# ucsd-hdsi-dvs/V2CE-Toolbox

Measured on AMD Instinct MI355X. Metric: frame-pairs/sec end-to-end (UNet+LDATI), 346x260, higher is better.
Workload: dtype f32-as-f16x2 (operands split hi/lo in fp16, 3 MFMAs per product, f32 accumulate)

## Files before the change

### v2ce-toolbox_amd/csrc/conv3d_wt.hip

```cpp
#include "conv3d_dev.h"
#include "conv3d_host.h"

#include <algorithm>
#include <cstdlib>
#include <map>
#include <mutex>
#include <tuple>
#include <vector>

namespace v2ce {
namespace {

constexpr int kWtSlot = 256;
constexpr int kWtChs = 4 * kWtSlot;
constexpr int kWtTaps = 36;

template <int CO_FR, int PO_FR, int RES, bool TAIL = false>
__global__ __launch_bounds__(512, 1) void conv3d_wt_kernel(ConvParams P) {
#if defined(__HIP_DEVICE_COMPILE__)
    [[maybe_unused]] unsigned long long t_all = TICK(), t_bar = 0, t_epi = 0, t_xbar = 0, t_cvt = 0, t_e0 = 0, t_e1 = 0, t_e2 = 0;
    static_assert(PO_FR == 4, "the output transform hands position fragment f to consumer wave f");
    constexpr bool PEPI = !TAIL;
    constexpr int CK = 16, NA = 3, CO_TILE = CO_FR * 32, chs = kWtChs;
    f16x8 *pieces = reinterpret_cast<f16x8 *>(conv_smem);
    float *aff = reinterpret_cast<float *>(conv_smem + (size_t)2 * 4 * chs * 16);

    const int tid = threadIdx.x, lane = tid & 63, l32 = lane & 31, half = lane >> 5;
    const int wave = __builtin_amdgcn_readfirstlane(tid >> 6);
    const int CG = P.Cin / CK;
    const long long wplane = (long long)kWtTaps * CG * P.Cout * 16;

    struct TileId { int b, co_t, t0, h0, w0, s0; };
    auto decode = [&](int vb, TileId &T) -> bool {
        const int xcd = vb & 7, q = vb >> 3;
        T.co_t = P.xcd_remap == 2 ? q / P.per_xcd : q % P.n_co_tiles;
        const int sp = P.xcd_remap == 2 ? q - T.co_t * P.per_xcd : q / P.n_co_tiles;
        int bid = xcd * P.per_xcd + sp;
        if (sp >= P.per_xcd || bid >= P.n_spatial) return false;
        const int iw = bid % P.nW;            bid /= P.nW;
        const int ih = bid % P.nH;            bid /= P.nH;
        const int it = bid % P.nT;            bid /= P.nT;
        T.b = bid;
        T.t0 = it * P.TT; T.h0 = ih * P.TH; T.w0 = iw * P.TW; T.s0 = 0;
        if (P.flat) { T.s0 = iw * P.flat; T.h0 = T.s0 / P.Wout; T.w0 = 0; }
        return true;
    };
    auto pos_of = [&](int m, const TileId &T, int &pp, int &th, int &tw) -> bool {
        if (P.flat) {
            pp = m / P.flat;
            const int s = T.s0 + (m - pp * P.flat);
            const int h = s / P.Wout;
            th = h - T.h0;
            tw = s - h * P.Wout;
            return m < P.n_pos && s < P.Hout * P.Wout;
        }
        pp = m / (P.TH * P.TW);
        const int rem = m - pp * (P.TH * P.TW);
        th = rem / P.TW;
        tw = rem - th * P.TW;
        return m < P.n_pos;
    };
    auto next_tile = [&](int &vb, TileId &T) -> bool {
        for (; vb < P.total_blocks; vb += (int)gridDim.x)
            if (decode(vb, T)) return true;
        return false;
    };

    const float *tail = reinterpret_cast<const float *>(P.wq + 2 * wplane);
    const float w_scale = tail[1];
    auto amax_of = [&](int b) -> float { return P.x0_absmax ? P.x0_absmax[b * P.amax_bs] : 4094.0f; };
    auto scale_of = [&](int b) -> float { return P.x0_absmax ? pow2_prescale(2.0f * amax_of(b)) : 0.5f * kActScale; };
    const int NTB = TAIL ? P.tCG / 4 : 0;
    const int CGT = CG + NTB;
    auto tamax_of = [&](int b) -> float {
        if (!P.tx0_absmax) return 4094.0f;
        float am = P.tx0_absmax[b * P.amax_bs];
        if (P.tx1_absmax) am = fmaxf(am, P.tx1_absmax[b * P.amax_bs]);
        return am;
    };
    auto tscale_of = [&](int b) -> float { return P.tx0_absmax ? pow2_prescale(tamax_of(b)) : kActScale; };
    const float wt_scale = TAIL ? reinterpret_cast<const float *>(P.sc_w + 2 * (long long)P.tCG * P.Cout * 16)[1] : 1.0f;
    auto acc_scale_of = [&](int b) -> float { return TAIL ? fminf(scale_of(b) * w_scale, tscale_of(b) * wt_scale) : scale_of(b) * w_scale; };
    auto xs_of = [&](int b) -> float { return TAIL ? acc_scale_of(b) / w_scale : scale_of(b); };
    auto ts_of = [&](int b) -> float { return acc_scale_of(b) / wt_scale; };
    const int nI = CG < NTB ? CG : NTB;
    auto is_tail = [&](int k) -> bool { return TAIL && (k < 2 * nI ? (k & 1) != 0 : NTB > CG); };
    auto idx_of = [&](int k) -> int { return !TAIL ? k : (k < 2 * nI ? k >> 1 : k - nI); };
    if (P.guard && blockIdx.x == 0 && wave == 0) {
        float sm = 0.0f;
        for (int co = lane; co < P.Cout; co += 64) sm = fmaxf(sm, fabsf(P.scale[co]));
#pragma unroll
        for (int o = 32; o; o >>= 1) sm = fmaxf(sm, __shfl_xor(sm, o));
        const int nb = P.amax_bs ? P.B : 1;
        for (int b = lane; b < nb; b += 64) {
            const float am = 2.0f * amax_of(b), xs = xs_of(b);
            float E = sm * (float)(P.Cin * 27) * 0x1p-25f * (tail[0] / xs + am / tail[1]);
            if (TAIL) {
                const float *tl = reinterpret_cast<const float *>(P.sc_w + 2 * (long long)P.tCG * P.Cout * 16);
                const float tam = tamax_of(b), txs = ts_of(b);
                E += sm * (float)(P.tCG * 16) * 0x1p-25f * (tl[0] / txs + tam / tl[1]);
                if (!(xs > 0x1p-100f && txs > 0x1p-100f)) E = __builtin_inff();
            }
            P.guard[b * P.amax_bs] = E;
        }
    }

    int vb = blockIdx.x;
    TileId T;
    if (!next_tile(vb, T)) return;
    int gc = 0;
    struct Pos { int pp, th, tw; bool ok; };
    auto pos_cached = [&](int m) -> Pos {
        Pos q{0, 0, 0, false};
        if (!P.flat) q.ok = pos_of(m, T, q.pp, q.th, q.tw);
        return q;
    };
    auto pos_get = [&](const Pos &c, int m, const TileId &L) -> Pos {
        if (!P.flat) return c;
        Pos q;
        q.ok = pos_of(m, L, q.pp, q.th, q.tw);
        return q;
    };

    if (wave >= 4) {
        const int ptid = tid - 256;
        const bool wave_on = (wave - 4) * 64 < P.plane;
        const int e_pp = ptid / (P.HH * P.HWd), e_hh = (ptid - e_pp * (P.HH * P.HWd)) / P.HWd, e_hw = ptid - e_pp * (P.HH * P.HWd) - e_hh * P.HWd;
        const Pos tpos = pos_cached(ptid & 127);
        float x_scale = xs_of(T.b);
        float t_scale = TAIL ? ts_of(T.b) : 1.0f;
        TileId Tprev = T;
        unsigned toff[2][2];
        [[maybe_unused]] int tm_pp = 0, tm_hi = 0, tm_wi = 0, tm_hs = 0, tm_ws = 0;
        [[maybe_unused]] bool tm_ok = false;
        __amdgpu_buffer_rsrc_t rs_t0 = __builtin_amdgcn_make_buffer_rsrc(const_cast<float *>(P.x0), 0, 0, 0x00020000), rs_t1 = rs_t0;
        unsigned goff[4];
        float R0[4][CK], R1[4][CK];
        __amdgpu_buffer_rsrc_t rs_in = __builtin_amdgcn_make_buffer_rsrc(const_cast<float *>(P.x0), 0, 0, 0x00020000);
        const long long seq = (long long)P.T * P.Cin * (P.Hin * P.Winp);
        const int cg_bytes = P.Hin * P.Winp * 64;
        auto load_chunk = [&](const TileId &L, int kseq, float (&R)[4][CK]) {
            const int cidx = idx_of(kseq);
            if (is_tail(kseq)) {
                typedef float f32x4g __attribute__((ext_vector_type(4)));
                if (cidx == 0) {
#pragma unroll
                    for (int sidx = 0; sidx < 2; ++sidx) toff[sidx][0] = toff[sidx][1] = kOOB;
                    if (tm_ok) {
                        {
                            const int hi = tm_hi, wi = tm_wi, hs = tm_hs, ws = tm_ws, pp = tm_pp;
#pragma unroll
                            for (int i = 0; i < 2; ++i) {
                                const int t = L.t0 + 2 * pp + i;
                                if (t < P.T) {
                                    toff[0][i] = 4u * (unsigned)((t * P.tC0) * (P.tH0 * P.tW0p)) + 64u * (unsigned)(hs * P.tW0p + ws);
                                    toff[1][i] = 4u * (unsigned)((t * P.tC1) * (P.tHin * P.tWinp)) + 64u * (unsigned)(hi * P.tWinp + wi);
                                }
                            }
                        }
                    }
                    const long long seq0 = (long long)P.T * P.tC0 * (P.tH0 * P.tW0p), seq1 = (long long)P.T * P.tC1 * (P.tHin * P.tWinp);
                    rs_t0 = __builtin_amdgcn_make_buffer_rsrc(const_cast<float *>(P.tx0 + L.b * seq0), 0, (int)(seq0 * 4), 0x00020000);
                    rs_t1 = __builtin_amdgcn_make_buffer_rsrc(const_cast<float *>(P.tx1 ? P.tx1 + L.b * seq1 : P.tx0), 0, P.tx1 ? (int)(seq1 * 4) : 0, 0x00020000);
                }
                const int gs = (wave - 4) >> 1;
                const int CG0 = P.tC0 / 16;
#pragma unroll
                for (int hb = 0; hb < 2; ++hb) {
                    const int g = hb * (P.tCG / 2) + 2 * cidx + gs;
                    const bool s1 = g >= CG0;
                    const int gbytes = s1 ? (g - CG0) * (P.tHin * P.tWinp * 64) : g * (P.tH0 * P.tW0p * 64);
#pragma unroll
                    for (int i = 0; i < 2; ++i)
#pragma unroll
                        for (int k4 = 0; k4 < CK / 4; ++k4) {
                            const f32x4g v = s1 ? __builtin_bit_cast(f32x4g, __builtin_amdgcn_raw_buffer_load_b128(rs_t1, toff[1][i], gbytes + 16 * k4, 0))
                                                : __builtin_bit_cast(f32x4g, __builtin_amdgcn_raw_buffer_load_b128(rs_t0, toff[0][i], gbytes + 16 * k4, 0));
                            R[2 * hb + i][4 * k4] = v[0]; R[2 * hb + i][4 * k4 + 1] = v[1]; R[2 * hb + i][4 * k4 + 2] = v[2]; R[2 * hb + i][4 * k4 + 3] = v[3];
                        }
                }
                return;
            }
            if (cidx == 0) {
                if constexpr (TAIL) {
                    const Pos q = pos_get(tpos, ptid & 127, L);
                    tm_ok = q.ok && L.h0 + q.th < P.Hout && L.w0 + q.tw < P.Wout;
                    tm_pp = q.pp;
                    tm_hi = tm_ok ? (L.h0 + q.th) * P.tS : 0;
                    tm_wi = tm_ok ? (L.w0 + q.tw) * P.tS : 0;
                    tm_hs = P.thmap ? P.thmap[tm_hi] : tm_hi;
                    tm_ws = P.twmap ? P.twmap[tm_wi] : tm_wi;
                }
#pragma unroll
                for (int i = 0; i < 4; ++i) goff[i] = kOOB;
                if (ptid < P.plane) {
                    const int pp = e_pp, hh = e_hh, hw = e_hw;
                    const int h = L.h0 - 1 + hh, w = L.w0 - 1 + hw;
                    if (h >= 0 && h < P.Hin && w >= 0 && w < P.Win) {
#pragma unroll
                        for (int i = 0; i < 4; ++i) {
                            const int t = L.t0 + 2 * pp - 1 + i;
                            if (t >= 0 && t < P.T) goff[i] = 4u * (unsigned)((t * P.Cin) * (P.Hin * P.Winp)) + 64u * (unsigned)(h * P.Winp + w);
                        }
                    }
                }
                rs_in = __builtin_amdgcn_make_buffer_rsrc(const_cast<float *>(P.x0 + L.b * seq), 0, (int)(seq * 4), 0x00020000);
            }
            if (wave_on) {
                typedef float f32x4g __attribute__((ext_vector_type(4)));
#pragma unroll
                for (int i = 0; i < 4; ++i)
#pragma unroll
                    for (int k4 = 0; k4 < CK / 4; ++k4) {
#if defined(V2CE_ABLATE_TAPS) && (V2CE_ABLATE_TAPS & 4)
                        if (k4) { R[i][4 * k4] = R[i][0]; R[i][4 * k4 + 1] = R[i][1]; R[i][4 * k4 + 2] = R[i][2]; R[i][4 * k4 + 3] = R[i][3]; continue; }
#endif
                        const f32x4g v = __builtin_bit_cast(f32x4g, __builtin_amdgcn_raw_buffer_load_b128(rs_in, goff[i], cidx * cg_bytes + 16 * k4, 0));
                        R[i][4 * k4] = v[0]; R[i][4 * k4 + 1] = v[1]; R[i][4 * k4 + 2] = v[2]; R[i][4 * k4 + 3] = v[3];
                    }
            }
        };
        int vbL = vb, cgL = 0;
        TileId TL = T;
        bool moreL = true;
        auto load_next = [&](float (&R)[4][CK]) {
            if (!moreL) return;
            load_chunk(TL, cgL, R);
            if (++cgL == CGT) {
                cgL = 0;
                vbL += (int)gridDim.x;
                moreL = next_tile(vbL, TL);
            }
        };
        int cgC = 0;
        auto convert_with = [&](float c_scale0, float c_scale12, auto tf) __attribute__((always_inline)) {
            f16x8 *qb = pieces + (gc & 1) * 4 * chs;
#pragma unroll
            for (int j = 0; j < 4; ++j) {
                const float c_scale = (j == 1 || j == 2) ? c_scale12 : c_scale0;
#pragma unroll
                for (int hg = 0; hg < 2; ++hg) {
                    typedef unsigned u32x4c __attribute__((ext_vector_type(4)));
                    u32x4c ph, pl;
#pragma unroll
                    for (int c2 = 0; c2 < 4; ++c2) {
                        const float xa = tf(j, 8 * hg + 2 * c2), xb = tf(j, 8 * hg + 2 * c2 + 1);
                        unsigned h, l;
                        asm("v_fma_mixlo_f16 %0, %2, %4, 0\n\t"
                            "v_fma_mixhi_f16 %0, %3, %4, 0\n\t"
                            "v_fma_mixlo_f16 %1, %2, %4, -%0 op_sel_hi:[0,0,1]\n\t"
                            "v_fma_mixhi_f16 %1, %3, %4, -%0 op_sel:[0,0,1] op_sel_hi:[0,0,1]"
                            : "=&v"(h), "=&v"(l) : "v"(xa), "v"(xb), "v"(c_scale));
                        ph[c2] = h;
                        pl[c2] = l;
                    }
                    qb[hg * chs + j * kWtSlot + ptid] = __builtin_bit_cast(f16x8, ph);
                    qb[(2 + hg) * chs + j * kWtSlot + ptid] = __builtin_bit_cast(f16x8, pl);
                }
            }
        };
        auto convert = [&](const float (&R)[4][CK]) {
            const bool tail = is_tail(cgC);
            if (!wave_on && !tail) return;
            [[maybe_unused]] const unsigned long long tcv = TICK();
            if (tail) {
                convert_with(t_scale, 0.5f * t_scale, [&](int j, int c) -> float {
                    return j == 0 ? R[0][c] : j == 1 ? R[2][c] + R[3][c] : j == 2 ? R[2][c] - R[3][c] : -R[1][c];
                });
            } else {
                convert_with(x_scale, x_scale, [&](int j, int c) -> float {
                    return j == 0 ? R[0][c] - R[2][c] : j == 1 ? R[1][c] + R[2][c] : j == 2 ? R[2][c] - R[1][c] : R[1][c] - R[3][c];
                });
            }
            ACC_T(t_cvt, tcv);
        };
        bool moreC = true;
        auto advance = [&]() {
            ++gc;
            if (++cgC == CGT) {
                cgC = 0;
                Tprev = T;
                vb += (int)gridDim.x;
                moreC = next_tile(vb, T);
                if (moreC) {
                    x_scale = xs_of(T.b);
                    if (TAIL) t_scale = ts_of(T.b);
                }
            }
        };
        const int fr = wave - 4;
        int spk;
        {
            const Pos q = pos_cached(fr * 32 + l32);
            spk = q.ok ? (q.pp << 20) | (q.th << 10) | q.tw : -1;
        }
        int seen_b = -1;
        unsigned seen_max = 0u;
        int ntile_p = 0;
        auto tile_rendezvous = [&]() {
            [[maybe_unused]] const unsigned long long tb = TICK();
            if constexpr (!PEPI) {
#pragma unroll
                for (int k = 0; k < 2 * CO_FR; ++k) lds_barrier();
                ACC_T(t_xbar, tb);
                return;
            }
            typedef float f32x4t __attribute__((ext_vector_type(4)));
            typedef unsigned u32x4t __attribute__((ext_vector_type(4)));
            const TileId &E = Tprev;
            const int co0 = E.co_t * CO_TILE;
            const float out_inv_scale = 1.0f / acc_scale_of(E.b);
            const float *a2 = aff + (ntile_p & 1) * 2 * CO_TILE;
            ++ntile_p;
            int poff[2], roff[2];
            {
                const int m = fr * 32 + l32;
// ... 202 lines not shown
        if constexpr (TAIL) {
#pragma unroll
            for (int f = 0; f < PO_FR; ++f) bpt[f] = half * chs + wave * kWtSlot + f * 32 + l32;
        }
        auto chunk_barrier = [&]() -> const f16x8 * {
            const f16x8 *qb = pieces + (gc & 1) * 4 * chs;
            [[maybe_unused]] const unsigned long long tb = TICK();
            __syncthreads();
            ACC_T(t_bar, tb);
            ++gc;
            return qb;
        };
        auto main_chunk = [&](int cg) __attribute__((always_inline)) {
            const f16x8 *qb = chunk_barrier();
                const int wc = slot_off + cg * cg_stride;
                const int wn = cg + 1 < CG ? wc + cg_stride : slot_off;
#pragma unroll
                for (int f = 0; f < PO_FR; ++f) {
                    bh[f] = qb[bhb[f]];
                    bl[f] = qb[bhb[f] + 2 * chs];
                }
                step_loop<0, 9>([&](auto tc) {
                    constexpr int tap = decltype(tc)::value;
                    constexpr int nt = tap + 1;
                    constexpr int dh = nt / 3, dw = nt % 3;
                    constexpr int pt = tap + NA - 1;
#if !(defined(V2CE_ABLATE_TAPS) && (V2CE_ABLATE_TAPS & 1))
                    if constexpr (pt < 9) {
                        V2CE_LOAD_A(pt % NA, wc + pt * tap_stride)
                    } else {
                        V2CE_LOAD_A(pt % NA, wn + (pt - 9) * tap_stride)
                    }
#endif
                    const int toff = dh * P.HWd + dw;
#pragma unroll
                    for (int f = 0; f < PO_FR; ++f) {
#pragma unroll
                        for (int q = 0; q < CO_FR; ++q) {
                            acc[q][f] = __builtin_amdgcn_mfma_f32_32x32x16_f16(ah[tap % NA][q], bh[f], acc[q][f], 0, 0, 0);
                            acc[q][f] = __builtin_amdgcn_mfma_f32_32x32x16_f16(ah[tap % NA][q], bl[f], acc[q][f], 0, 0, 0);
                            acc[q][f] = __builtin_amdgcn_mfma_f32_32x32x16_f16(al[tap % NA][q], bh[f], acc[q][f], 0, 0, 0);
                        }
#if !(defined(V2CE_ABLATE_TAPS) && (V2CE_ABLATE_TAPS & 2))
                        if constexpr (nt < 9) {
                            bh[f] = qb[bhb[f] + toff];
                            bl[f] = qb[bhb[f] + toff + 2 * chs];
                        }
#endif
                        __builtin_amdgcn_sched_barrier(0);
                    }
                });
        };
        auto tail_prefetch = [&](int kb) __attribute__((always_inline)) {
            const int w0 = (gbase + 2 * kb) * cg_stride;
#pragma unroll
            for (int q = 0; q < (TAIL ? CO_FR : 0); ++q) {
                ath[0][q] = __builtin_bit_cast(f16x8, __builtin_amdgcn_raw_buffer_load_b128(rs_t, wlane[q], w0, 0));
                atl[0][q] = __builtin_bit_cast(f16x8, __builtin_amdgcn_raw_buffer_load_b128(rs_t, wlane[q], w0 + (int)(2 * tplane), 0));
            }
        };
        auto tail_barrier = [&](int kb) __attribute__((always_inline)) {
            if constexpr (TAIL) {
                const f16x8 *qb = chunk_barrier();
                const int w1 = (gbase + 2 * kb + 1) * cg_stride;
#pragma unroll
                for (int q = 0; q < CO_FR; ++q) {
                    ath[1][q] = __builtin_bit_cast(f16x8, __builtin_amdgcn_raw_buffer_load_b128(rs_t, wlane[q], w1, 0));
                    atl[1][q] = __builtin_bit_cast(f16x8, __builtin_amdgcn_raw_buffer_load_b128(rs_t, wlane[q], w1 + (int)(2 * tplane), 0));
                }
#pragma unroll
                for (int gs = 0; gs < 2; ++gs) {
#pragma unroll
                    for (int f = 0; f < PO_FR; ++f) {
                        bh[f] = qb[bpt[f] + gs * 128];
                        bl[f] = qb[bpt[f] + gs * 128 + 2 * chs];
                    }
#pragma unroll
                    for (int f = 0; f < PO_FR; ++f)
#pragma unroll
                        for (int q = 0; q < CO_FR; ++q) {
                            acc[q][f] = __builtin_amdgcn_mfma_f32_32x32x16_f16(ath[gs][q], bh[f], acc[q][f], 0, 0, 0);
                            acc[q][f] = __builtin_amdgcn_mfma_f32_32x32x16_f16(ath[gs][q], bl[f], acc[q][f], 0, 0, 0);
                            acc[q][f] = __builtin_amdgcn_mfma_f32_32x32x16_f16(atl[gs][q], bh[f], acc[q][f], 0, 0, 0);
                        }
                }
            }
        };
        if constexpr (!TAIL) {
            for (int cg = 0; cg < CG; ++cg) main_chunk(cg);
        } else {
            for (int i = 0; i < nI; ++i) {
                main_chunk(i);
                tail_prefetch(i);
                tail_barrier(i);
            }
            for (int i = nI; i < CG; ++i) main_chunk(i);
            for (int i = nI; i < NTB; ++i) {
                tail_prefetch(i);
                tail_barrier(i);
            }
        }

        if constexpr (PEPI) {
        [[maybe_unused]] const unsigned long long te = TICK();
        typedef float f32x4t __attribute__((ext_vector_type(4)));
        f32x4t *xch = reinterpret_cast<f32x4t *>(pieces + ((gc - 1) & 1) * 4 * chs);
#pragma unroll
        for (int q = 0; q < CO_FR; ++q) {
#pragma unroll
            for (int f = 0; f < PO_FR; ++f)
#pragma unroll
                for (int r4 = 0; r4 < 4; ++r4) {
                    f32x4t v;
                    v[0] = acc[q][f][4 * r4]; v[1] = acc[q][f][4 * r4 + 1]; v[2] = acc[q][f][4 * r4 + 2]; v[3] = acc[q][f][4 * r4 + 3];
                    xch[f * chs + wave * kWtSlot + r4 * 64 + lane] = v;
                }
            [[maybe_unused]] const unsigned long long tb = TICK();
            lds_barrier();
            lds_barrier();
            ACC_T(t_xbar, tb);
        }
        ACC_T(t_epi, te);
        } else {
        const float *aff_c = aff + ((ntile - 1) & 1) * 2 * CO_TILE;
// ... 94 lines not shown
                    ACC_T(t_xbar, tb);
                    te2 = TICK();
                }
#pragma unroll
                for (int rr = 0; rr < 2; ++rr) {
                    const int r4 = 2 * hp + rr;
#pragma unroll
                    for (int o = 0; o < 2; ++o) {
                        f32x4t out;
#pragma unroll
                        for (int k = 0; k < 4; ++k) {
                            const float y = o == 0 ? (mm[rr][0][k] + mm[rr][1][k]) + mm[rr][2][k] : (mm[rr][1][k] - mm[rr][2][k]) - mm[rr][3][k];
                            float v = y * (scq[r4][k] * inv_scale) + shq[r4][k];
                            v += rv[o][r4][k];
                            v = apply_act(v, slope);
                            out[k] = v;
                            const unsigned av = __builtin_bit_cast(unsigned, v) & vmask[o];
                            ymax = av > ymax ? av : ymax;
                        }
                        __builtin_amdgcn_raw_buffer_store_b128(__builtin_bit_cast(u32x4t, out), rs_y, vo[o], soff(r4), 0);
                        asm volatile("s_nop 1" : "+v"(out));
                    }
                }
            }
        }
        if (P.y_absmax) {
#pragma unroll
            for (int o = 32; o; o >>= 1) {
                const unsigned other = (unsigned)__shfl_xor((int)ymax, o);
                ymax = other > ymax ? other : ymax;
            }
            if (T.b != seen_b) { seen_b = T.b; seen_max = 0u; }
            if (ymax > seen_max) {
                seen_max = ymax;
                if (lane == 0) atomicMax(reinterpret_cast<unsigned *>(P.y_absmax + T.b * P.amax_bs), ymax);
            }
        }
        ACC_T(t_epi, te);
        ACC_T(t_e2, te2);
        }
        vb += (int)gridDim.x;
        more = next_tile(vb, T);
    }
#ifdef V2CE_STAMP
    if (lane == 0 && wave == 0) {
        unsigned long long *o = P.stamps + ((long long)blockIdx.x * 2 + 0) * 8;
        o[0] = TICK() - t_all; o[1] = t_bar; o[2] = t_xbar; o[3] = t_epi; o[4] = (unsigned long long)gc; o[5] = t_e0; o[6] = t_e1; o[7] = t_e2;
    }
#endif
#undef V2CE_LOAD_A
#endif
}

constexpr int kWtMaxBatch = 16;
struct WtLayer {
    const float *w, *sigma;
    _Float16 *packed;
    int rows, cin;
    int cin_total, ci0;
    long long tail_halves;
};
struct WtBatch {
    WtLayer L[kWtMaxBatch];
    int n;
    int blk[kWtMaxBatch + 1];
};
constexpr size_t kWtPackLds = (size_t)32 * 432 * 4 + (size_t)2 * kWtTaps * 514 * 2;

template <int PASS>
__global__ __launch_bounds__(512) void wt_pack_kernel(WtBatch B) {
    extern __shared__ __attribute__((aligned(16))) unsigned char wt_smem[];
    float *wf = reinterpret_cast<float *>(wt_smem);
    _Float16 *hi = reinterpret_cast<_Float16 *>(wt_smem + 32 * 432 * 4), *lo = hi + kWtTaps * 514;
    int l = 0;
    while (l + 1 < B.n && (int)blockIdx.x >= B.blk[l + 1]) ++l;
    const WtLayer &P = B.L[l];
    const int CG = P.cin / 16;
    const int blk = blockIdx.x - B.blk[l];
    const int cg = blk % CG, co0 = (blk / CG) * 32;
    const long long n = (long long)P.rows * P.cin * kWtTaps;
    float *tail = reinterpret_cast<float *>(P.packed + P.tail_halves);
    const float sigma = P.sigma ? P.sigma[0] : 1.0f;
    for (int e = threadIdx.x; e < 32 * 432; e += 512) {
        const int col = e / 432, rem = e - col * 432;
        wf[e] = P.w[((long long)(co0 + col) * P.cin_total + P.ci0 + cg * 16) * 27 + rem] / sigma;
    }
    __syncthreads();
    const float w_scale = PASS ? pow2_prescale(tail[0]) : 1.0f;
    if (PASS && blk == 0 && threadIdx.x == 0) tail[1] = w_scale;
    float m = 0.0f;
    for (int it = threadIdx.x; it < 32 * 16 * 9; it += 512) {
        const int col = it / 144, rem = it - col * 144, j = rem / 9, t9 = rem - j * 9;
        const float *g = wf + col * 432 + j * 27 + t9;
        const float g0 = g[0], g1 = g[9], g2 = g[18];
        float G[4];
        G[0] = g0;
        G[1] = ((g0 + g1) + g2) * 0.5f;
        G[2] = ((g0 - g1) + g2) * 0.5f;
        G[3] = g2;
        if (!PASS) {
            m = fmaxf(m, fmaxf(fabsf(g0), fmaxf(fabsf(g1), fabsf(g2))));
            continue;
        }
#pragma unroll
        for (int s = 0; s < 4; ++s) {
            const float v = G[s] * w_scale;
// ... 30 lines not shown
    if (B.blk[B.n] == 0) return V2CE_OK;
    if (pass == 0) hipLaunchKernelGGL(wt_pack_kernel<0>, dim3(B.blk[B.n]), dim3(512), kWtPackLds, st, B);
    else hipLaunchKernelGGL(wt_pack_kernel<1>, dim3(B.blk[B.n]), dim3(512), kWtPackLds, st, B);
    V2CE_HIP_CHECK(hipGetLastError());
    return V2CE_OK;
}

struct WtBox { int pp, th, tw, flat; };

WtBox choose_wt_box(int B, int T, int H, int W, int n_co, int n_cu, int pos_tile) {
    if (const char *e = getenv("V2CE_WT_BOX")) {
        WtBox b{0, 0, 0, 0};
        if (sscanf(e, "%d,%d,%d", &b.pp, &b.th, &b.tw) == 3 && b.pp > 0 && b.th > 0 && b.tw > 0 && b.pp * b.th * b.tw <= pos_tile &&
            b.pp * (b.th + 2) * (b.tw + 2) <= kWtSlot)
            return b;
    }
    static std::mutex mu;
    static std::map<std::tuple<int, int, int, int, int, int>, WtBox> cache;
    std::lock_guard<std::mutex> g(mu);
    const auto key = std::make_tuple(B, T, H, W, n_co, pos_tile);
    auto it = cache.find(key);
    if (it != cache.end()) return it->second;
    const int pairs = (T + 1) / 2;
    WtBox best{0, 0, 0, 0};
    double best_cost = 1e30;
    for (int pp = 1; pp <= pairs && pp <= 16; ++pp) {
        const int n_max = pos_tile / pp;
        if (n_max < 1) break;
        const int nR = (H * W + n_max - 1) / n_max, n = (H * W + nR - 1) / nR;
        const int rows = std::min(H, (W - 1 + n - 1) / W + 1);
        if (pp * (rows + 2) * (W + 2) > kWtSlot) continue;
        const long long nsp = (long long)B * ((pairs + pp - 1) / pp) * nR;
        const long long blocks = 8 * ((nsp + 7) / 8) * n_co;
        const double rounds = (double)((blocks + n_cu - 1) / n_cu);
        const double halo = (double)pp * (rows + 2) * (W + 2) / kWtSlot;
        const double cost = rounds * (1.0 + 0.15 * halo) + 1e-3 * (double)blocks / n_cu;
        if (cost < best_cost) { best_cost = cost; best = WtBox{pp, rows, W, n}; }
    }
    for (int pp = 1; pp <= pairs && pp <= 16; ++pp)
        for (int th = 1; th <= H && th <= 64; ++th)
            for (int tw = 1; tw <= W && tw <= 128; ++tw) {
                if (pp * th * tw > pos_tile || pp * (th + 2) * (tw + 2) > kWtSlot) continue;
                const long long nsp = (long long)B * ((pairs + pp - 1) / pp) * ((H + th - 1) / th) * ((W + tw - 1) / tw);
                const long long blocks = 8 * ((nsp + 7) / 8) * n_co;
                const double rounds = (double)((blocks + n_cu - 1) / n_cu);
                const double halo = (double)pp * (th + 2) * (tw + 2) / kWtSlot;
                const double cost = rounds * (1.0 + 0.15 * halo) + 1e-3 * (double)blocks / n_cu;
                if (cost < best_cost - 1e-9) { best_cost = cost; best = WtBox{pp, th, tw, 0}; }
            }
    cache.emplace(key, best);
    return best;
}

template <int CO_FR, int PO_FR, int RES, bool TAIL = false>
int launch_wt(ConvParams P, const v2ce_conv3d_desc &d, hipStream_t stream) {
    constexpr int CO_TILE = CO_FR * 32, POS_TILE = PO_FR * 32;
    if (g_name_out) {
        snprintf(g_name_out, g_name_cap, "conv3d_wt_kernel<%d,%d,%d,%d>", CO_FR, PO_FR, RES, (int)TAIL);
        return V2CE_OK;
    }
    P.n_co_tiles = (d.Cout + CO_TILE - 1) / CO_TILE;
    WtBox bx{d.tile_t / 2, d.tile_h, d.tile_w, 0};
    if (bx.pp <= 0 || bx.th <= 0 || bx.tw <= 0) bx = choose_wt_box(d.B, d.T, d.Hout, d.Wout, P.n_co_tiles, persistent_cu_count(), POS_TILE);
    V2CE_REQUIRE(bx.pp > 0 && bx.th > 0 && bx.tw > 0, V2CE_ERR_UNSUPPORTED, "v2ce_conv3d_fwd_wt: no box fits");
    P.TT = 2 * bx.pp; P.TH = bx.th; P.TW = bx.tw;
    P.flat = bx.flat;
    P.n_pos = bx.flat ? bx.pp * bx.flat : bx.pp * bx.th * bx.tw;
    P.HT = bx.pp; P.HH = bx.th + 2; P.HWd = bx.tw + 2;
    P.plane = P.HT * P.HH * P.HWd;
    P.nT = (d.T + P.TT - 1) / P.TT; P.nH = (d.Hout + bx.th - 1) / bx.th; P.nW = (d.Wout + bx.tw - 1) / bx.tw;
    if (bx.flat) { P.nH = 1; P.nW = (d.Hout * d.Wout + bx.flat - 1) / bx.flat; }
    V2CE_REQUIRE(P.n_pos <= POS_TILE && P.plane <= kWtSlot, V2CE_ERR_UNSUPPORTED, "v2ce_conv3d_fwd_wt: tile does not fit");
    P.n_spatial = d.B * P.nT * P.nH * P.nW;
    P.per_xcd = (P.n_spatial + 7) / 8;
    const double w_bytes = (double)CO_TILE * P.Cin * kWtTaps * 4, x_bytes = (double)P.per_xcd * P.n_pos * 2 * P.Cin * 4;
    P.xcd_remap = P.n_co_tiles > 1 && w_bytes * P.n_co_tiles > x_bytes ? 2 : 1;
    const long long blocks = (long long)8 * P.per_xcd * P.n_co_tiles;
    P.total_blocks = (int)blocks;
    const size_t lds = (size_t)kWtChs * (2 * 4 * 16) + 2 * 2 * CO_TILE * sizeof(float);
    auto kern = conv3d_wt_kernel<CO_FR, PO_FR, RES, TAIL>;
    static const int once = [&] {
        (void)hipFuncSetAttribute(reinterpret_cast<const void *>(kern), hipFuncAttributeMaxDynamicSharedMemorySize, (int)lds);
        return 0;
    }();
    (void)once;
    if (getenv("V2CE_WT_VERBOSE"))
        fprintf(stderr, "[wt<%d,%d,%d%s> %dx%dx%dx%d C %d -> %d] box %d pairs x %d x %d%s (%d of %d positions, %d halo elements), %lld tiles\n", CO_FR, PO_FR, RES, TAIL ? ",tail" : "", d.B, d.T,
                d.Hout, d.Wout, P.Cin, P.Cout, bx.pp, bx.th, bx.tw, bx.flat ? " rows: flat ranges" : "", P.n_pos, POS_TILE, P.plane, blocks);
    const unsigned grid = persistent_grid(blocks);
#ifdef V2CE_STAMP
    V2CE_HIP_CHECK(hipMalloc(&P.stamps, (size_t)grid * 16 * sizeof(unsigned long long)));
    V2CE_HIP_CHECK(hipMemset(P.stamps, 0, (size_t)grid * 16 * sizeof(unsigned long long)));
#endif
    hipLaunchKernelGGL(kern, dim3(grid), dim3(512), lds, stream, P);
    V2CE_HIP_CHECK(hipGetLastError());
#ifdef V2CE_STAMP
    {
        std::vector<unsigned long long> h((size_t)grid * 16);
        V2CE_HIP_CHECK(hipDeviceSynchronize());
        V2CE_HIP_CHECK(hipMemcpy(h.data(), P.stamps, h.size() * 8, hipMemcpyDeviceToHost));
        V2CE_HIP_CHECK(hipFree(P.stamps));
        auto mean = [&](int role, int a) {
            double sm = 0;
            for (unsigned k = 0; k < grid; ++k) sm += (double)h[((size_t)k * 2 + role) * 8 + a];
            return sm / grid;
        };
        const double tot = mean(0, 0), chunks = mean(0, 4), tiles = chunks / (P.Cin / 16);
        fprintf(stderr, "[stamp wt<%d,%d,%d> C %d -> %d %dx%d box %dx%dx%d] per workgroup: %.1f tiles, %.0f chunks, %.0f cycles (s_memtime, 100 MHz) | consumer: chunk barriers %.1f %%, "
                "epilogue %.1f %% (its barriers %.1f %%), main loop %.1f %% = %.1f ticks per chunk | producer: chunk barriers %.1f %%, rendezvous %.1f %%, convert %.1f %%\n",
                CO_FR, PO_FR, RES, P.Cin, P.Cout, d.Hout, d.Wout, bx.pp, bx.th, bx.tw, tiles, chunks, tot, 100 * mean(0, 1) / tot, 100 * mean(0, 3) / tot,
                100 * mean(0, 2) / tot, 100 * (tot - mean(0, 1) - mean(0, 3)) / tot, (tot - mean(0, 1) - mean(0, 3)) / chunks, 100 * mean(1, 1) / mean(1, 0),
                100 * mean(1, 2) / mean(1, 0), 100 * mean(1, 3) / mean(1, 0));
        fprintf(stderr, "    epilogue per tile (cycles): loads + dump (incl. the previous round's compute and stores) %.0f, first barrier .. reads %.0f, last compute + stores + range %.0f, barriers %.0f\n",
                mean(0, 5) / tiles, mean(0, 6) / tiles, mean(0, 7) / tiles, mean(0, 2) / tiles);
    }
#endif
    return V2CE_OK;
}

struct WtTail {
    const v2ce_conv3d_desc *desc;
    const float *tx0, *tx1;
    const int *thmap, *twmap;
    const void *w;
    const float *tx0_absmax, *tx1_absmax;
    int res_h, res_wp;
};

int wt_dispatch(const v2ce_conv3d_desc *desc, const float *x, const void *w_wt, const float *scale, const float *shift,
                const float *residual, float *y, const float *x_absmax, float *y_absmax, v2ce_stream_t stream, const WtTail *tl = nullptr) {
    clear_error();
    V2CE_REQUIRE(desc && (g_name_out || (x && w_wt && scale && shift && y)), V2CE_ERR_BAD_ARG, "v2ce_conv3d_fwd_wt: null pointer");
    const v2ce_conv3d_desc &d = *desc;
    V2CE_REQUIRE(d.B > 0 && d.T > 0 && d.C0 > 0 && d.C1 == 0 && d.Hin > 0 && d.Win > 0 && d.Cout > 0, V2CE_ERR_BAD_ARG,
                 "v2ce_conv3d_fwd_wt: bad shape (one source: C1 must be 0)");
    V2CE_REQUIRE(d.ksize == 3 && d.stride_hw == 1 && d.precision == V2CE_PRECISION_F16X2 && d.layout == V2CE_LAYOUT_C16, V2CE_ERR_UNSUPPORTED,
                 "v2ce_conv3d_fwd_wt: a split-half 3x3x3 stride-1 conv on channels-last-16 activations");
    V2CE_REQUIRE(d.H0 == d.Hin && d.W0 == d.Win && d.Hout == d.Hin && d.Wout == d.Win, V2CE_ERR_BAD_ARG, "v2ce_conv3d_fwd_wt: input and output planes must have one size");
    V2CE_REQUIRE(d.C0 % 16 == 0 && d.Cout % 64 == 0, V2CE_ERR_UNSUPPORTED, "v2ce_conv3d_fwd_wt: Cin must be a multiple of 16, Cout of 64");
    V2CE_REQUIRE(d.act >= 0 && d.act <= 2, V2CE_ERR_BAD_ARG, "v2ce_conv3d_fwd_wt: act %d", d.act);
    V2CE_REQUIRE(g_name_out || (aligned16(x, w_wt, residual, y) && (!tl || aligned16(tl->tx0, tl->tx1, tl->w))), V2CE_ERR_BAD_ARG,
                 "v2ce_conv3d_fwd_wt: weight buffers and channels-last-16 tensors must be 16-byte aligned");
    const int Winp = d.W0_pitch > 0 ? d.W0_pitch : d.W0, Woutp = d.Wout_pitch > 0 ? d.Wout_pitch : d.Wout;
    V2CE_REQUIRE(Winp >= d.Win && Woutp >= d.Wout, V2CE_ERR_BAD_ARG, "v2ce_conv3d_fwd_wt: a row pitch is smaller than its width");
    V2CE_REQUIRE((long long)d.T * d.C0 * d.Hin * Winp < (1ll << 29) && (long long)d.T * d.Cout * d.Hout * Woutp < (1ll << 29), V2CE_ERR_UNSUPPORTED,
                 "v2ce_conv3d_fwd_wt: a single sequence exceeds the 2 GiB buffer-descriptor range");
    V2CE_REQUIRE(v2ce_pack_weights_f16x2_wt_bytes(d.Cout, d.C0) < (1ull << 31), V2CE_ERR_UNSUPPORTED,
                 "v2ce_conv3d_fwd_wt: the weight buffer exceeds the 2 GiB buffer-descriptor range");
    ConvParams P{};
    P.x0 = x; P.scale = scale; P.shift = shift; P.res = residual; P.y = y;
    P.B = d.B; P.T = d.T; P.C0 = d.C0; P.H0 = d.H0; P.W0 = d.W0; P.Hin = d.Hin; P.Win = d.Win;
    P.Cin = d.C0; P.Cout = d.Cout; P.Hout = d.Hout; P.Wout = d.Wout;
    P.W0p = Winp; P.Winp = Winp; P.Woutp = Woutp;
    P.c16 = 1;
    P.act = d.act;
    P.wq = static_cast<const _Float16 *>(w_wt);
    P.x0_absmax = x_absmax; P.y_absmax = y_absmax;
    P.guard = y_absmax ? y_absmax + 1 : nullptr;
    P.amax_bs = d.absmax_batch_stride;
    V2CE_REQUIRE(P.amax_bs == 0 || P.amax_bs >= 2, V2CE_ERR_BAD_ARG, "v2ce_conv3d_fwd_wt: absmax_batch_stride must be 0 or >= 2");
    hipStream_t st = as_stream(stream);
    if (tl) {
        V2CE_REQUIRE(tl->desc && tl->w, V2CE_ERR_BAD_ARG, "v2ce_conv3d_fwd_wt_tail: null tail description / weights");
        if (residual && tl->res_h > 0) {
            V2CE_REQUIRE(tl->res_h == (d.Hout + 1) / 2 && tl->res_wp >= (d.Wout + 1) / 2, V2CE_ERR_BAD_ARG,
                         "v2ce_conv3d_fwd_wt_tail: an upsampled residual has ceil(Hout / 2) rows of at least ceil(Wout / 2) columns");
            V2CE_REQUIRE((long long)d.T * d.Cout * tl->res_h * tl->res_wp < (1ll << 29), V2CE_ERR_UNSUPPORTED, "v2ce_conv3d_fwd_wt_tail: residual too large");
            P.res_up = 1; P.rH = tl->res_h; P.rWp = tl->res_wp;
        }
        const v2ce_conv3d_desc &t = *tl->desc;
        V2CE_REQUIRE(t.ksize == 1 && (t.stride_hw == 1 || t.stride_hw == 2) && t.layout == V2CE_LAYOUT_C16 && t.B == d.B && t.T == d.T &&
                     t.Cout == d.Cout && t.Hout == d.Hout && t.Wout == d.Wout && t.C0 > 0 && t.C0 % 16 == 0 && t.C1 >= 0 &&
                     t.C1 % 16 == 0 && t.Hout == (t.Hin - 1) / t.stride_hw + 1 && t.Wout == (t.Win - 1) / t.stride_hw + 1,
                     V2CE_ERR_BAD_ARG, "v2ce_conv3d_fwd_wt_tail: the tail must be a 1x1x1 conv (channels-last-16, channel counts multiples "
                     "of 16) producing exactly the main conv's output shape");
        V2CE_REQUIRE(((t.C0 + t.C1) / 16) % 4 == 0, V2CE_ERR_UNSUPPORTED, "v2ce_conv3d_fwd_wt_tail: the tail's channel count must be a multiple of 64");
        V2CE_REQUIRE((g_name_out || tl->tx0) && (t.C1 == 0 || tl->tx1 || g_name_out) && (tl->thmap == nullptr) == (tl->twmap == nullptr) &&
                     (tl->thmap || (t.H0 == t.Hin && t.W0 == t.Win)), V2CE_ERR_BAD_ARG, "v2ce_conv3d_fwd_wt_tail: tail inputs / index maps");
        V2CE_REQUIRE((tl->tx0_absmax != nullptr) == (x_absmax != nullptr) && (t.C1 == 0 || !tl->tx0_absmax || tl->tx1_absmax), V2CE_ERR_BAD_ARG,
                     "v2ce_conv3d_fwd_wt_tail: range slots of the tail inputs");
        P.tx0 = tl->tx0; P.tx1 = t.C1 > 0 ? tl->tx1 : nullptr; P.thmap = tl->thmap; P.twmap = tl->twmap;
        P.tC0 = t.C0; P.tH0 = t.H0; P.tW0p = t.W0_pitch > 0 ? t.W0_pitch : t.W0; P.tC1 = t.C1; P.tHin = t.Hin; P.tWin = t.Win;
        P.tWinp = t.Win_pitch > 0 ? t.Win_pitch : t.Win; P.tS = t.stride_hw; P.tCG = (t.C0 + t.C1) / 16;
        P.tx0_absmax = tl->tx0_absmax; P.tx1_absmax = t.C1 > 0 ? tl->tx1_absmax : nullptr;
        P.sc_w = static_cast<const _Float16 *>(tl->w);
        V2CE_REQUIRE((long long)t.T * t.C0 * t.H0 * P.tW0p < (1ll << 29) && (long long)t.T * t.C1 * t.Hin * P.tWinp < (1ll << 29),
                     V2CE_ERR_UNSUPPORTED, "v2ce_conv3d_fwd_wt_tail: a single sequence exceeds the 2 GiB buffer-descriptor range");
        if (residual) return launch_wt<2, 4, 1, true>(P, d, st);
        return launch_wt<2, 4, 0, true>(P, d, st);
    }
    if (residual || (g_name_out && scale)) return launch_wt<2, 4, 1>(P, d, st);
    return launch_wt<2, 4, 0>(P, d, st);
}

}

int v2ce_wt_pack_batch(const float *const *w, const float *const *sigma, void *const *packed, const int *rows, const int *cin, int n, int pass,
                       hipStream_t st, const int *cin_total, const int *ci0) {
    V2CE_REQUIRE(n >= 0 && n <= kWtMaxBatch, V2CE_ERR_BAD_ARG, "v2ce_wt_pack_batch: 0..%d layers", kWtMaxBatch);
    WtBatch B{};
    B.n = n;
    for (int l = 0; l < n; ++l) {
        V2CE_REQUIRE(rows[l] % 32 == 0 && cin[l] % 16 == 0, V2CE_ERR_UNSUPPORTED, "v2ce_wt_pack_batch: Cout %% 32, Cin %% 16");
        B.L[l] = WtLayer{w[l], sigma[l], static_cast<_Float16 *>(packed[l]), rows[l], cin[l], cin_total ? cin_total[l] : cin[l], ci0 ? ci0[l] : 0,
                         2ll * rows[l] * cin[l] * kWtTaps};
        if (pass == 0) {
            B.L[l].cin = B.L[l].cin_total;
            B.L[l].ci0 = 0;
        }
        V2CE_REQUIRE(B.L[l].ci0 >= 0 && B.L[l].ci0 + cin[l] <= B.L[l].cin_total, V2CE_ERR_BAD_ARG, "v2ce_wt_pack_batch: channel slice out of range");
        B.blk[l + 1] = B.blk[l] + (rows[l] / 32) * (B.L[l].cin / 16);
    }
    if (n == 0) return V2CE_OK;
    return wt_pack_launch(B, pass, st);
}

}

using namespace v2ce;

extern "C" size_t v2ce_pack_weights_f16x2_wt_bytes(int Cout, int Cin) {
    if (Cout <= 0 || Cin <= 0) return 0;
    return (size_t)2 * kWtTaps * Cout * Cin * sizeof(_Float16) + 16;
}

extern "C" int v2ce_pack_weights_f16x2_wt_slice(const float *w, int Cout, int Cin_total, int ci0, int Cin, const float *sigma, void *w_wt,
                                                v2ce_stream_t stream) {
    clear_error();
    V2CE_REQUIRE(w && w_wt && Cout > 0 && Cin > 0 && ci0 >= 0 && ci0 + Cin <= Cin_total, V2CE_ERR_BAD_ARG, "v2ce_pack_weights_f16x2_wt: bad argument");
    V2CE_REQUIRE(Cout % 32 == 0 && Cin % 16 == 0 && ci0 % 16 == 0, V2CE_ERR_UNSUPPORTED,
                 "v2ce_pack_weights_f16x2_wt: Cout must be a multiple of 32, the channel slice of 16");
    hipStream_t st = as_stream(stream);
    unsigned char *tail = static_cast<unsigned char *>(w_wt) + (size_t)2 * kWtTaps * Cout * Cin * sizeof(_Float16);
    V2CE_HIP_CHECK(hipMemsetAsync(tail, 0, 16, st));
    void *pk = w_wt;
    int rc = v2ce_wt_pack_batch(&w, &sigma, &pk, &Cout, &Cin, 1, 0, st, &Cin_total, &ci0);
    if (rc != V2CE_OK) return rc;
    return v2ce_wt_pack_batch(&w, &sigma, &pk, &Cout, &Cin, 1, 1, st, &Cin_total, &ci0);
}

// ... 44 lines not shown
```

### v2ce-toolbox_amd/v2ce_3d.py

```python
from __future__ import annotations

import ctypes
import os
from collections import OrderedDict

import numpy as np
import torch
import torch.nn as nn

from . import hip

BN_EPS = 1e-5
BASE, NUM_ENC, NUM_RES = 32, 4, 2


class _Conv(nn.Module):

    def __init__(self, cin, cout, k, bias):
        super().__init__()
        w = torch.empty(cout, cin, k, k, k)
        nn.init.kaiming_normal_(w, 10.0)
        self.weight = nn.Parameter(w, requires_grad=False)
        if bias:
            self.bias = nn.Parameter(torch.zeros(cout), requires_grad=False)
# ... 163 lines not shown
        dev = self.UNet.head.conv3d.weight.device
        if dev.type != "cuda":
            raise hip.V2ceHipError("V2ce3d: parameters must be on a HIP device (.to('cuda')); "
                                   "there is no CPU path")
        for p in self.parameters():
            if p.dtype != torch.float32:
                raise hip.V2ceHipError("V2ce3d: parameters must be float32")
        P = {}
        ones = lambda c: torch.ones(c, dtype=torch.float32, device=dev)
        h = self.UNet.head.conv3d
        P["head"] = (self._pack(h.weight.contiguous()), ones(h.weight.shape[0]), h.bias.float().contiguous())
        P["head_split"] = None
        if (self.precision == "f16x2" and tuple(h.weight.shape) in ((32, 2, 3, 3, 3), (32, 3, 3, 3, 3))
                and os.environ.get("V2CE_HEAD_SPLIT", "1") != "0"):
            sfx = "_c3" if h.weight.shape[1] == 3 else ""
            tab = torch.empty(getattr(hip.lib(), f"v2ce_pack_head_weights_f16x2{sfx}_bytes")() // 2, dtype=torch.float16, device=dev)
            hip.check(getattr(hip.lib(), f"v2ce_pack_head_weights_f16x2{sfx}")(h.weight.contiguous().data_ptr(), tab.data_ptr(),
                                                                                hip.stream_ptr(dev)),
                      f"v2ce_pack_head_weights_f16x2{sfx}")
            P["head_split"] = (tab, h.bias.float().contiguous())
        pr = self.UNet.pred.conv3d
        P["pred"] = (self._pack(pr.weight.contiguous()), ones(pr.weight.shape[0]), pr.bias.float().contiguous())
        P["pred_fused"] = None
        if self.precision == "f16x2" and pr.weight.shape[1] == 32 and pr.weight.shape[0] <= 32:
            tab = torch.empty(hip.lib().v2ce_pack_pred_weights_f16x2_bytes() // 2, dtype=torch.float16, device=dev)
            hip.check(hip.lib().v2ce_pack_pred_weights_f16x2(pr.weight.contiguous().data_ptr(), pr.weight.shape[0], 32,
                                                             tab.data_ptr(), hip.stream_ptr(dev)),
                      "v2ce_pack_pred_weights_f16x2")
            bias = torch.zeros(32, dtype=torch.float32, device=dev)
            bias[:pr.weight.shape[0]] = pr.bias.float()
            P["pred_fused"] = (tab, bias, int(pr.weight.shape[0]))
        sn_ws = 0
        for name, blocks in (("enc", self.UNet.encoders), ("res", self.UNet.resblocks),
                             ("dec", self.UNet.decoders)):
            for i, blk in enumerate(blocks):
                d = {}
                splits = {"conv1": self._split(blk.cin, blk.cout), "conv2": self._split(blk.cout, blk.cout)}
                d["bn1"] = self._fold_bn(blk.bn1)
                d["bn2"] = self._fold_bn(blk.bn2)
                d["down_w"] = self._pack(blk.downsample[0].weight.contiguous(),
                                         split=self._fuse_shortcut(blk) or self._split(blk.cin, blk.cout, 1, blk.stride_hw))
                d["down_bn"] = self._fold_bn(blk.downsample[1], blk.downsample[0].bias)
                d["fold"] = None
                if self._fold_shortcut(blk):
                    s2, sh2 = d["bn2"]
                    sd, shd = d["down_bn"]
                    if float(s2.abs().min()) > 1e-20 and bool(torch.isfinite(sd / s2).all()):
                        wf = (blk.downsample[0].weight * (sd / s2).view(-1, 1, 1, 1, 1)).contiguous()
                        d["fold"] = (self._pack(wf, split=True), s2, (sh2 + shd).contiguous())
                        d["fold_w32"] = wf
                wt = {"conv1": self._winograd() and splits["conv1"] and name == "res" and blk.stride_hw == 1 and blk.cout % 64 == 0
                      and not self._fuse_shortcut(blk),
                      "conv2": self._winograd() and splits["conv2"] and blk.cout % 64 == 0 and
                      (d["fold"] is None or (blk.cin % 64 == 0 and os.environ.get("V2CE_WT_TAIL", "1") != "0"))}
                d["wt"] = wt
                d["fold_lo"] = d["fold_skip"] = None
                if name == "dec" and d["fold"] is not None and self._upfold() and os.environ.get("V2CE_TAIL_LOWRES", "1") != "0" and \
                        wt["conv2"] and (blk.cin // 3) % 64 == 0:
                    c0 = blk.cin * 2 // 3
                    wf = (blk.downsample[0].weight * (d["down_bn"][0] / d["bn2"][0]).view(-1, 1, 1, 1, 1))
                    d["fold_lo"] = self._pack(wf[:, :c0].contiguous(), split=True)
                    d["fold_skip_w32"] = wf[:, c0:].contiguous()
                    d["fold_skip"] = self._pack(d["fold_skip_w32"], split=True)
                d["zero_shift"] = torch.zeros(blk.cout, dtype=torch.float32, device=dev)
                if blk.sn:
                    for cn in ("conv1", "conv2"):
                        m = getattr(blk, cn).module
                        rows, cols = m.weight_bar.shape[0], m.weight_bar[0].numel()
                        up_c0 = blk.cin * 2 // 3 if (name == "dec" and cn == "conv1" and self._upfold()) else 0
                        d[cn + "_w"] = (self._split_buffer(rows, m.weight_bar.shape[1], 27, dev, up_c0=up_c0, wt=wt[cn])
                                        if splits[cn] else torch.empty(rows * cols, dtype=torch.float32, device=dev))
                        if up_c0 and self._up_split(blk):
                            sk = self._split_buffer(rows, m.weight_bar.shape[1] - up_c0, 27, dev, wt=True)
                            sk.ci0 = up_c0
                            d["conv1_skip_w"] = sk
                            d["zero_shift"] = torch.zeros(rows, dtype=torch.float32, device=dev)
                        sn_ws = max(sn_ws, hip.lib().v2ce_sn_workspace_bytes(rows, cols))
                else:
                    for cn in ("conv1", "conv2"):
                        w = getattr(blk, cn).weight.contiguous()
                        out = self._split_buffer(w.shape[0], w.shape[1], 27, dev, wt=True) if wt[cn] else None
                        d[cn + "_w"] = self._pack(w, out=out, split=splits[cn])
                P[f"{name}{i}"] = d
        P["sn_ws"] = torch.empty(max(sn_ws, 16), dtype=torch.uint8, device=dev)
        P["sigma"] = torch.empty(1, dtype=torch.float32, device=dev)
        P["sn_batch"] = None
        if self.precision == "f16x2":
            inners = [(getattr(blk, cn).module, P[f"{name}{i}"][cn + "_w"], P[f"{name}{i}"].get("conv1_skip_w") if cn == "conv1" else None)
                      for name, blocks in (("res", self.UNet.resblocks), ("dec", self.UNet.decoders))
                      for i, blk in enumerate(blocks) if blk.sn for cn in ("conv1", "conv2")]
            arr = (hip.SnLayer * len(inners))()
            for e, (m, out, skip) in zip(arr, inners):
                e.w_bar, e.u, e.v, e.packed = m.weight_bar.data_ptr(), m.weight_u.data_ptr(), m.weight_v.data_ptr(), out.data_ptr()
                e.rows, e.cols, e.k3 = m.weight_bar.shape[0], m.weight_bar[0].numel(), 27
                e.up_c0 = getattr(out, "up_c0", 0)
                e.wt = 1 if getattr(out, "wt", False) else 0
                e.packed_skip = None if skip is None else skip.data_ptr()
            nb = hip.lib().v2ce_sn_batch_workspace_bytes(arr, len(inners))
            if nb:
                P["sn_batch"] = (arr, len(inners), torch.empty(nb, dtype=torch.uint8, device=dev))
            P["sn_once"] = None
            if nb and os.environ.get("V2CE_SN_REPACK", "0") != "1":
                one = torch.ones(1, dtype=torch.float32, device=dev)
                inv_sigma = torch.ones(len(inners), dtype=torch.float32, device=dev)
                keep, tails, k = [one, inv_sigma], [], 0
                for name, blocks in (("res", self.UNet.resblocks), ("dec", self.UNet.decoders)):
                    for i, blk in enumerate(blocks):
# ... 594 lines not shown
```

Before: 4015.

## Support Winograd conv with fused shortcut tail for 32-multiple channel counts

Adds an ODD variant of the Winograd conv kernel whose fused 1x1x1 shortcut tail processes one 16-channel group per step instead of two. This lets layers whose shortcut input has a channel count that is a multiple of 32 but not 64 use the fused Winograd path. Before, those layers fell back to a non-Winograd or unfused path. Half the tail loader waves and converter waves sit idle in the odd case, and the change adds another kernel instantiation.

```diff
diff --git a/v2ce-toolbox_amd/csrc/conv3d_wt.hip b/v2ce-toolbox_amd/csrc/conv3d_wt.hip
--- a/v2ce-toolbox_amd/csrc/conv3d_wt.hip
+++ b/v2ce-toolbox_amd/csrc/conv3d_wt.hip
@@ -15,8 +15,8 @@
 constexpr int kWtChs = 4 * kWtSlot;
 constexpr int kWtTaps = 36;
 
-template <int CO_FR, int PO_FR, int RES, bool TAIL = false>
-__global__ __launch_bounds__(512, 1) void conv3d_wt_kernel(ConvParams P) {
+template <int CO_FR, int PO_FR, int RES, bool TAIL, bool ODD>
+__device__ __forceinline__ void conv3d_wt_body(ConvParams P) {
 #if defined(__HIP_DEVICE_COMPILE__)
     [[maybe_unused]] unsigned long long t_all = TICK(), t_bar = 0, t_epi = 0, t_xbar = 0, t_cvt = 0, t_e0 = 0, t_e1 = 0, t_e2 = 0;
     static_assert(PO_FR == 4, "the output transform hands position fragment f to consumer wave f");
@@ -70,7 +70,9 @@
     const float w_scale = tail[1];
     auto amax_of = [&](int b) -> float { return P.x0_absmax ? P.x0_absmax[b * P.amax_bs] : 4094.0f; };
     auto scale_of = [&](int b) -> float { return P.x0_absmax ? pow2_prescale(2.0f * amax_of(b)) : 0.5f * kActScale; };
-    const int NTB = TAIL ? P.tCG / 4 : 0;
+    static_assert(TAIL || !ODD, "ODD describes the tail");
+    constexpr int KST = ODD ? 1 : 2;
+    const int NTB = TAIL ? P.tCG / (2 * KST) : 0;
     const int CGT = CG + NTB;
     auto tamax_of = [&](int b) -> float {
         if (!P.tx0_absmax) return 4094.0f;
@@ -164,10 +166,11 @@
                     rs_t1 = __builtin_amdgcn_make_buffer_rsrc(const_cast<float *>(P.tx1 ? P.tx1 + L.b * seq1 : P.tx0), 0, P.tx1 ? (int)(seq1 * 4) : 0, 0x00020000);
                 }
                 const int gs = (wave - 4) >> 1;
+                if (ODD && gs) return;
                 const int CG0 = P.tC0 / 16;
 #pragma unroll
                 for (int hb = 0; hb < 2; ++hb) {
-                    const int g = hb * (P.tCG / 2) + 2 * cidx + gs;
+                    const int g = hb * (P.tCG / 2) + KST * cidx + gs;
                     const bool s1 = g >= CG0;
                     const int gbytes = s1 ? (g - CG0) * (P.tHin * P.tWinp * 64) : g * (P.tH0 * P.tW0p * 64);
 #pragma unroll
@@ -262,6 +265,7 @@
         auto convert = [&](const float (&R)[4][CK]) {
             const bool tail = is_tail(cgC);
             if (!wave_on && !tail) return;
+            if (ODD && tail && wave >= 6) return;
             [[maybe_unused]] const unsigned long long tcv = TICK();
             if (tail) {
                 convert_with(t_scale, 0.5f * t_scale, [&](int j, int c) -> float {
@@ -570,7 +574,7 @@
                 });
         };
         auto tail_prefetch = [&](int kb) __attribute__((always_inline)) {
-            const int w0 = (gbase + 2 * kb) * cg_stride;
+            const int w0 = (gbase + KST * kb) * cg_stride;
 #pragma unroll
             for (int q = 0; q < (TAIL ? CO_FR : 0); ++q) {
                 ath[0][q] = __builtin_bit_cast(f16x8, __builtin_amdgcn_raw_buffer_load_b128(rs_t, wlane[q], w0, 0));
@@ -582,12 +586,12 @@
                 const f16x8 *qb = chunk_barrier();
                 const int w1 = (gbase + 2 * kb + 1) * cg_stride;
 #pragma unroll
-                for (int q = 0; q < CO_FR; ++q) {
+                for (int q = 0; q < (ODD ? 0 : CO_FR); ++q) {
                     ath[1][q] = __builtin_bit_cast(f16x8, __builtin_amdgcn_raw_buffer_load_b128(rs_t, wlane[q], w1, 0));
                     atl[1][q] = __builtin_bit_cast(f16x8, __builtin_amdgcn_raw_buffer_load_b128(rs_t, wlane[q], w1 + (int)(2 * tplane), 0));
                 }
 #pragma unroll
-                for (int gs = 0; gs < 2; ++gs) {
+                for (int gs = 0; gs < KST; ++gs) {
 #pragma unroll
                     for (int f = 0; f < PO_FR; ++f) {
                         bh[f] = qb[bpt[f] + gs * 128];
@@ -788,6 +792,16 @@
 #endif
 }
 
+template <int CO_FR, int PO_FR, int RES, bool TAIL = false>
+__global__ __launch_bounds__(512, 1) void conv3d_wt_kernel(ConvParams P) {
+    conv3d_wt_body<CO_FR, PO_FR, RES, TAIL, false>(P);
+}
+
+template <int CO_FR, int PO_FR, int RES>
+__global__ __launch_bounds__(512, 1) void conv3d_wt_tail1_kernel(ConvParams P) {
+    conv3d_wt_body<CO_FR, PO_FR, RES, true, true>(P);
+}
+
 constexpr int kWtMaxBatch = 16;
 struct WtLayer {
     const float *w, *sigma;
@@ -924,7 +938,7 @@
     return best;
 }
 
-template <int CO_FR, int PO_FR, int RES, bool TAIL = false>
+template <int CO_FR, int PO_FR, int RES, bool TAIL = false, bool ODD = false>
 int launch_wt(ConvParams P, const v2ce_conv3d_desc &d, hipStream_t stream) {
     constexpr int CO_TILE = CO_FR * 32, POS_TILE = PO_FR * 32;
     if (g_name_out) {
@@ -950,7 +964,9 @@
     const long long blocks = (long long)8 * P.per_xcd * P.n_co_tiles;
     P.total_blocks = (int)blocks;
     const size_t lds = (size_t)kWtChs * (2 * 4 * 16) + 2 * 2 * CO_TILE * sizeof(float);
-    auto kern = conv3d_wt_kernel<CO_FR, PO_FR, RES, TAIL>;
+    void (*kern)(ConvParams);
+    if constexpr (ODD) kern = conv3d_wt_tail1_kernel<CO_FR, PO_FR, RES>;
+    else kern = conv3d_wt_kernel<CO_FR, PO_FR, RES, TAIL>;
     static const int once = [&] {
         (void)hipFuncSetAttribute(reinterpret_cast<const void *>(kern), hipFuncAttributeMaxDynamicSharedMemorySize, (int)lds);
         return 0;
@@ -1046,7 +1062,8 @@
                      t.C1 % 16 == 0 && t.Hout == (t.Hin - 1) / t.stride_hw + 1 && t.Wout == (t.Win - 1) / t.stride_hw + 1,
                      V2CE_ERR_BAD_ARG, "v2ce_conv3d_fwd_wt_tail: the tail must be a 1x1x1 conv (channels-last-16, channel counts multiples "
                      "of 16) producing exactly the main conv's output shape");
-        V2CE_REQUIRE(((t.C0 + t.C1) / 16) % 4 == 0, V2CE_ERR_UNSUPPORTED, "v2ce_conv3d_fwd_wt_tail: the tail's channel count must be a multiple of 64");
+        V2CE_REQUIRE(((t.C0 + t.C1) / 16) % 2 == 0, V2CE_ERR_UNSUPPORTED, "v2ce_conv3d_fwd_wt_tail: the tail's channel count must be a multiple of 32");
+        const bool odd = ((t.C0 + t.C1) / 16) % 4 != 0;
         V2CE_REQUIRE((g_name_out || tl->tx0) && (t.C1 == 0 || tl->tx1 || g_name_out) && (tl->thmap == nullptr) == (tl->twmap == nullptr) &&
                      (tl->thmap || (t.H0 == t.Hin && t.W0 == t.Win)), V2CE_ERR_BAD_ARG, "v2ce_conv3d_fwd_wt_tail: tail inputs / index maps");
         V2CE_REQUIRE((tl->tx0_absmax != nullptr) == (x_absmax != nullptr) && (t.C1 == 0 || !tl->tx0_absmax || tl->tx1_absmax), V2CE_ERR_BAD_ARG,
@@ -1058,6 +1075,7 @@
         P.sc_w = static_cast<const _Float16 *>(tl->w);
         V2CE_REQUIRE((long long)t.T * t.C0 * t.H0 * P.tW0p < (1ll << 29) && (long long)t.T * t.C1 * t.Hin * P.tWinp < (1ll << 29),
                      V2CE_ERR_UNSUPPORTED, "v2ce_conv3d_fwd_wt_tail: a single sequence exceeds the 2 GiB buffer-descriptor range");
+        if (odd) return residual ? launch_wt<2, 4, 1, true, true>(P, d, st) : launch_wt<2, 4, 0, true, true>(P, d, st);
         if (residual) return launch_wt<2, 4, 1, true>(P, d, st);
         return launch_wt<2, 4, 0, true>(P, d, st);
     }
diff --git a/v2ce-toolbox_amd/v2ce_3d.py b/v2ce-toolbox_amd/v2ce_3d.py
--- a/v2ce-toolbox_amd/v2ce_3d.py
+++ b/v2ce-toolbox_amd/v2ce_3d.py
@@ -239,7 +239,7 @@
                 wt = {"conv1": self._winograd() and splits["conv1"] and name == "res" and blk.stride_hw == 1 and blk.cout % 64 == 0
                       and not self._fuse_shortcut(blk),
                       "conv2": self._winograd() and splits["conv2"] and blk.cout % 64 == 0 and
-                      (d["fold"] is None or (blk.cin % 64 == 0 and os.environ.get("V2CE_WT_TAIL", "1") != "0"))}
+                      (d["fold"] is None or (blk.cin % 32 == 0 and os.environ.get("V2CE_WT_TAIL", "1") != "0"))}
                 d["wt"] = wt
                 d["fold_lo"] = d["fold_skip"] = None
                 if name == "dec" and d["fold"] is not None and self._upfold() and os.environ.get("V2CE_TAIL_LOWRES", "1") != "0" and \
```

New measurement: 4005. No clear change (-0.3%).
